# worm-privacy/proof-of-burn

Hardware: AMD Instinct MI355X
Metric: proof_of_burn witnesses/sec (higher is better)
Workload: dtype u64 bit-sliced lanes + BN254 Fr (8x32-bit Montgomery)

## Files before the change

### proof_of_burn_amd/csrc/poseidon_wide.hpp

```cpp
#pragma once
#include "kernels_common.hpp"

extern __shared__ uint32_t g_lds[];

#define POSW_NONE 0xFFFFFFFFu

template <bool RIDE, bool FAULT = false> struct PosWideT {
    __amdgpu_buffer_rsrc_t rs;
    uint32_t slot4;
    bool act;
    bool actb;
    const uint32_t* ktab;
    uint32_t kbase;
    uint32_t w_of_f;
    uint32_t w_also;
    mutable Fr pl, pv; mutable uint32_t pw, bad;
    uint32_t fault_f; bool fault_me;
    bool fault_val;
    __device__ __forceinline__ void ride_init() { pl = pv = fr_zero(); pw = 0; bad = 0xFFFFFFFFu; }
    __device__ __forceinline__ void ride_resolve() const { if (!fr_eq(pl, pv) && pw < bad) bad = pw; POB_OPAQUE(bad); }
    __device__ __forceinline__ Fr ld(uint32_t f) const {
        Fr v; const uint32_t off = act ? (f << 11) + slot4 : 0xFFFFF000u;
#pragma unroll
        for (int k = 0; k < 8; k++) v.l[k] = (uint32_t)__builtin_amdgcn_raw_buffer_load_b32(rs, (int)(off + 256u * k), 0, 0);
        return v;
    }
    __device__ __forceinline__ Fr st(bool on, uint32_t f, const Fr& v_in, bool also = false) const {
        const uint32_t off = on ? (f << 11) + slot4 : 0xFFFFF000u;
        Fr v = v_in;
        if constexpr (FAULT) { if (fault_val && fault_me && on && f == fault_f) v.l[0] ^= 1u; }
        const uint32_t flip = (FAULT && !fault_val && fault_me && f == fault_f) ? 1u : 0u;
#pragma unroll
        for (int k = 0; k < 8; k++) __builtin_amdgcn_raw_buffer_store_b32((int)(k == 0 ? v.l[0] ^ flip : v.l[k]), rs, (int)(off + 256u * k), 0, 0);
        if constexpr (RIDE) {
            Fr l;
#pragma unroll
            for (int k = 0; k < 8; k++) l.l[k] = (uint32_t)__builtin_amdgcn_raw_buffer_load_b32(rs, (int)(off + 256u * k), 0, 0);
            POB_RIDE_BARRIER();
            ride_resolve();
            pl = l; pv = fr_sel(on, v, fr_zero()); pw = also ? w_also : f + w_of_f;
        }
        return v;
    }
    __device__ __forceinline__ Fr kc(uint32_t idx) const {
        Fr v; const uint32_t* q = ktab + (size_t)(idx - kbase) * 8;
#pragma unroll
        for (int k = 0; k < 8; k++) v.l[k] = q[k];
        return v;
    }
};
typedef PosWideT<false> PosWide;
__device__ __forceinline__ Fr posw_from(const Fr& v, uint32_t src_lane) {
    Fr r;
#pragma unroll
    for (int k = 0; k < 8; k++) r.l[k] = (uint32_t)__builtin_amdgcn_ds_bpermute((int)(src_lane << 2), (int)v.l[k]);
    return r;
}
__device__ __forceinline__ Fr posw_group_sum(Fr v, uint32_t lane) {
#pragma unroll
    for (uint32_t m = 2; m >= 1; m >>= 1) v = fr_add(v, posw_from(v, lane ^ m));
    return v;
}

struct PosWDesc { uint32_t base, pre, in2, in3, in4, sub, also; };
template <int T, class PW> __device__ __forceinline__ Fr posw_input(const GArgs& A, const PosWDesc& d, const PW& W, uint32_t e, bool act) {
    Fr x = fr_zero();
    if (e == 1) x = A.L->prefix[d.pre];
    uint32_t a2 = e == 2 ? d.in2 : 0u, a3 = e == 3 ? d.in3 : 0u, a4 = e == 4 ? d.in4 : 0u;
    POB_OPAQUE(a2); POB_OPAQUE(a3); POB_OPAQUE(a4);
    const uint32_t aj = a2 | a3 | a4;
    const uint32_t src = (act && e >= 2) ? aj : POSW_NONE;
    PosWideT<false> Wi; Wi.rs = W.rs; Wi.slot4 = W.slot4; Wi.act = src != POSW_NONE;
    const Fr v = Wi.ld(src);
    if (src != POSW_NONE) x = v;
    const uint32_t sub = (act && e == (uint32_t)T - 1) ? d.sub : POSW_NONE;
    Wi.act = sub != POSW_NONE;
    const Fr s = Wi.ld(sub);
    if (sub != POSW_NONE) x = fr_sub(x, s);
    return fr_sel(act, x, fr_zero());
}

template <int T, class PW> __device__ __forceinline__ Fr posw_sbox(const PW& W, bool act, uint32_t e, Fr x, uint32_t off, uint32_t cr) {
    const Fr x2 = fr_sqr_inl(x), x4 = fr_sqr_inl(x2), x5 = fr_mul_inl(x4, x);
    const uint32_t sg = off + 4 * e;
    W.st(act, sg + 1, x); W.st(act, sg + 2, x2); W.st(act, sg + 3, x4); W.st(act, sg, x5);
    Fr y = fr_add(x5, W.kc(cr + (act ? e : 0)));
    W.st(act, off + 5 * T + e, x5); y = W.st(act, off + 4 * T + e, y);
    W.st(act, off + 7 * T + e, y);
    return y;
}
template <int T, class PW> __device__ __forceinline__ void posw_full(const PW& W, uint32_t lane, uint32_t j, Fr& x, Fr& xb, uint32_t off, uint32_t cr, uint32_t mat) {
    const bool act = W.act, actb = W.actb;
    const Fr y = posw_sbox<T>(W, act, j, x, off, cr);
    Fr yb = fr_zero();
    if constexpr (T == 5) yb = posw_sbox<T>(W, actb, 4, xb, off, cr);
    const uint32_t jc = act ? j : 0, g0 = lane & ~3u;
    Fr acc = fr_zero(), accb = fr_zero();
#pragma unroll 1
    for (uint32_t i = 0; i < (uint32_t)(T < 4 ? T : 4); i++) {
        const Fr yi = posw_from(y, g0 | i);
        acc = fr_add(acc, fr_mul_inl(W.kc(mat + jc * T + i), yi));
        if constexpr (T == 5) accb = fr_add(accb, fr_mul_inl(W.kc(mat + 4 * T + i), yi));
    }
    if constexpr (T == 5) {
        const Fr yi = posw_from(yb, g0 | 1u);
        acc = fr_add(acc, fr_mul_inl(W.kc(mat + jc * T + 4), yi));
        accb = fr_add(accb, fr_mul_inl(W.kc(mat + 4 * T + 4), yi));
        xb = W.st(actb, off + 6 * T + 4, accb);
    }
    x = W.st(act, off + 6 * T + j, acc);
}

template <int T, class PW> __device__ __forceinline__ void posw_run(const GArgs& A, const PosWDesc& d, const PW& W, uint32_t lane) {
    const PosOff k = pos_off(T);
    const uint32_t j = lane & 3u, base = d.base, g0 = lane & ~3u;
    const bool act = W.act, actb = W.actb, l0 = j == 0;
    const uint32_t jc = act ? j : 0;
    Fr x = posw_input<T>(A, d, W, j, act), xb = fr_zero();
    W.st(act && !l0, base + j, x);
    W.st(act && !l0, base + T + j, x);
    W.st(act && l0, base + 2 * T, x);
    W.st(act, base + 3 * T + 1 + j, x);
    x = fr_add(x, W.kc(k.C + jc));
    x = W.st(act, base + 2 * T + 1 + j, x);
    if constexpr (T == 5) {
        xb = posw_input<T>(A, d, W, 4, actb);
        W.st(actb, base + 4, xb); W.st(actb, base + T + 4, xb); W.st(actb, base + 3 * T + 5, xb);
        xb = fr_add(xb, W.kc(k.C + 4));
        xb = W.st(actb, base + 2 * T + 5, xb);
    }
    uint32_t off = base + 4 * T + 1;
#pragma unroll 1
    for (uint32_t r = 0; r < 4; r++) { posw_full<T>(W, lane, j, x, xb, off, k.C + (r + 1) * T, r == 3 ? k.Pm : k.M); off += 8 * T; }
    Fr pin0 = fr_zero();
    uint32_t poff = 0;
#pragma unroll 1
    for (uint32_t r = 0; r < (uint32_t)k.rp; r++) {
        const uint32_t sb = k.S + (2 * T - 1) * r;
        const Fr c1 = W.kc(sb + jc);
        const Fr m1 = fr_mul_inl(x, fr_sel(l0, x, c1));
        Fr m2, m3;
        if constexpr (T == 5) {
            const Fr cp = W.kc(r ? sb - (2 * T - 1) + T + 3 : sb);
            m2 = fr_mul_inl(fr_sel(l0, m1, pin0), fr_sel(l0, m1, cp));
            if (r) { xb = fr_add(xb, m2); xb = W.st(actb, poff + 4 + 4, xb); }
            m3 = fr_mul_inl(fr_sel(l0, m2, xb), fr_sel(l0, x, W.kc(sb + 4)));
        } else {
            m2 = fr_sqr_inl(m1);
            m3 = fr_mul_inl(m2, x);
        }
        const Fr s0 = fr_add(m3, W.kc(k.C + 5 * T + r));
        W.st(act && l0, off + 1, x); W.st(act && l0, off + 2, m1); W.st(act && l0, off + 3, m2); W.st(act && l0, off, m3);
        W.st(act, off + 4 + T + j, fr_sel(l0, s0, x));
        if constexpr (T == 5) W.st(actb, off + 4 + T + 4, xb);
        const Fr in0 = posw_from(s0, g0);
        const Fr c2 = W.kc(jc == 0 ? sb : sb + T + jc - 1);
        const Fr m4 = fr_mul_inl(c2, in0);
        Fr part = fr_sel(l0, m4, m1);
        if constexpr (T == 5) if (actb) part = fr_add(part, m3);
        if (!act) part = fr_zero();
        const Fr sum = posw_group_sum(part, lane);
        x = fr_sel(l0, sum, fr_add(x, m4));
        x = W.st(act, off + 4 + j, x);
        if constexpr (T == 5) { pin0 = in0; poff = off; }
        off += 4 + 2 * T;
    }
    if constexpr (T == 5) {
        xb = fr_add(xb, fr_mul_inl(pin0, W.kc(k.S + (2 * T - 1) * (k.rp - 1) + T + 3)));
        xb = W.st(actb, poff + 4 + 4, xb);
    }
#pragma unroll 1
    for (uint32_t r = 0; r < 3; r++) { posw_full<T>(W, lane, j, x, xb, off, k.C + 5 * T + k.rp + r * T, k.M); off += 8 * T; }
    {
        const Fr x2 = fr_sqr_inl(x), x4 = fr_sqr_inl(x2), x5 = fr_mul_inl(x4, x);
        const uint32_t sg = off + 4 * j;
        W.st(act, sg + 1, x); W.st(act, sg + 2, x2); W.st(act, sg + 3, x4); W.st(act, sg, x5);
        W.st(act, off + 4 * T + 1 + j, x5);
        Fr part = fr_mul_inl(W.kc(k.M + jc), x5);
        if constexpr (T == 5) {
            const Fr b2 = fr_sqr_inl(xb), b4 = fr_sqr_inl(b2), b5 = fr_mul_inl(b4, xb);
            W.st(actb, off + 17, xb); W.st(actb, off + 18, b2); W.st(actb, off + 19, b4); W.st(actb, off + 16, b5);
            W.st(actb, off + 4 * T + 5, b5);
            const Fr pb = fr_mul_inl(W.kc(k.M + 4), b5);
            if (actb) part = fr_add(part, pb);
        }
        if (!act) part = fr_zero();
        const Fr h = posw_group_sum(part, lane);
        W.st(act && l0, off + 4 * T, h);
        W.st(act && l0, base + T, h);
        W.st(act && l0, base, h);
        W.st(act && l0 && d.also != POSW_NONE, d.also, h, true);
    }
}

#define POSW_SLICES 4
#ifndef POSW_WAVES
#define POSW_WAVES 4
#endif
static_assert(POSW_SLICES % POSW_WAVES == 0, "the slices of a workgroup belong to one unit");
template <bool RIDE, bool FAULT = false> __device__ __forceinline__ void poswide_body(const GArgs& A, uint32_t bx, uint32_t g) {
    __builtin_amdgcn_s_setprio(3);
    const uint32_t lane = threadIdx.x & 63u;
    const UnitDesc* dp = A.units + POB_UNI(A.order[A.first + bx / POSW_SLICES]);
    const int T = (int)POB_UNI(dp->a[0]);
    const PosWDesc d = {POB_UNI(dp->cur.f), POB_UNI(dp->a[1]), POB_UNI(dp->a[2]), POB_UNI(dp->a[3]), POB_UNI(dp->a[4]), POB_UNI(dp->a[5]), POB_UNI(dp->a[6])};
    const PosOff k = pos_off(T);
    const uint32_t kend = T == 3 ? POS_OFF_C_4 : T == 4 ? POS_OFF_C_5 : POS_TABLE_LEN;
    for (uint32_t i = threadIdx.x; i < (kend - k.C) * 8; i += blockDim.x) g_lds[i] = A.pos_tab[(size_t)k.C * 8 + i];
    __syncthreads();
    PosWideT<RIDE, FAULT> W;
    uint32_t* frp = A.fr + (uint64_t)g * A.fr_stride;
    const uint64_t nf = A.fr_stride * 4;
    W.rs = __builtin_amdgcn_make_buffer_rsrc(frp, 0, (int)(nf > 0xFFFFF000ull ? 0xFFFFF000ull : nf), 0x00020000);
    const uint32_t slot = 16 * (bx % POSW_SLICES) + (lane >> 2);
    W.slot4 = slot * 4;
    W.act = (lane & 3u) < (uint32_t)T;
    W.actb = T == 5 && (lane & 3u) == 1;
    W.ktab = g_lds; W.kbase = k.C;
    W.w_of_f = POB_UNI(dp->cur.w) - d.base; W.w_also = POB_UNI(dp->cur.w);
    if constexpr (RIDE) W.ride_init();
    if constexpr (FAULT) { W.fault_f = A.fault_idx; W.fault_me = (A.fault_cls & 0xFFu) == 2 && g == A.fault_group && ((A.fault_lanes >> slot) & 1); W.fault_val = (A.fault_cls & FAULT_VALUE) != 0; }
    if (T == 3) posw_run<3>(A, d, W, lane); else if (T == 4) posw_run<4>(A, d, W, lane); else posw_run<5>(A, d, W, lane);
    if constexpr (RIDE) {
        W.ride_resolve();
        uint32_t b = W.bad;
#pragma unroll
        for (uint32_t m = 2; m >= 1; m >>= 1) { const uint32_t o = (uint32_t)__builtin_amdgcn_ds_bpermute((int)((lane ^ m) << 2), (int)b); b = o < b ? o : b; }
        if ((lane & 3u) == 0 && b != 0xFFFFFFFFu) atomicMin(&A.bad_wire[g * 64 + slot], b);
    }
}
template <bool RIDE, bool FAULT> __global__ void __launch_bounds__(64 * POSW_WAVES) k_poseidon_wide(GArgs A) { poswide_body<RIDE, FAULT>(A, POSW_WAVES * blockIdx.x + (threadIdx.x >> 6), blockIdx.y); }
static_assert(POS_TABLE_LEN - POS_OFF_C_5 >= POS_OFF_C_5 - POS_OFF_C_4 && POS_TABLE_LEN - POS_OFF_C_5 >= POS_OFF_C_4 - POS_OFF_C_3, "the T = 5 constants are the largest set");
#define POSW_LDS_BYTES ((POS_TABLE_LEN - POS_OFF_C_5) * 32u)
```

Before: 1.230 million.

## Batch Poseidon wide stores and readbacks through a four-slot ring, spread lane-4 work via DPP

Replaces the per-store write-then-readback verification with a 4-entry ring of pending stores. Readbacks are issued in batches and their comparisons resolved later, so load latency overlaps with the following arithmetic. The lone T=5 fifth-element lane's stores are redistributed across the quad using DPP quad permutes, so all four lanes issue stores in parallel instead of one lane serialising them. This adds register pressure from the ring state and intricate slot bookkeeping, and fault and ride-check attribution now depends on the ring indices being correct.

```diff
diff --git a/proof_of_burn_amd/csrc/poseidon_wide.hpp b/proof_of_burn_amd/csrc/poseidon_wide.hpp
--- a/proof_of_burn_amd/csrc/poseidon_wide.hpp
+++ b/proof_of_burn_amd/csrc/poseidon_wide.hpp
@@ -5,6 +5,8 @@
 
 #define POSW_NONE 0xFFFFFFFFu
 
+#define POSW_OFF 0xFFFFF000u
+#define POSW_RING 4
 template <bool RIDE, bool FAULT = false> struct PosWideT {
     __amdgpu_buffer_rsrc_t rs;
     uint32_t slot4;
@@ -14,33 +16,64 @@
     uint32_t kbase;
     uint32_t w_of_f;
     uint32_t w_also;
-    mutable Fr pl, pv; mutable uint32_t pw, bad;
+    mutable Fr pl[POSW_RING], pv[POSW_RING]; mutable uint32_t po[POSW_RING], bad;
     uint32_t fault_f; bool fault_me;
     bool fault_val;
-    __device__ __forceinline__ void ride_init() { pl = pv = fr_zero(); pw = 0; bad = 0xFFFFFFFFu; }
-    __device__ __forceinline__ void ride_resolve() const { if (!fr_eq(pl, pv) && pw < bad) bad = pw; POB_OPAQUE(bad); }
+    __device__ __forceinline__ void ride_init() {
+#pragma unroll
+        for (int i = 0; i < POSW_RING; i++) { pl[i] = pv[i] = fr_zero(); po[i] = POSW_OFF; }
+        bad = 0xFFFFFFFFu;
+    }
     __device__ __forceinline__ Fr ld(uint32_t f) const {
-        Fr v; const uint32_t off = act ? (f << 11) + slot4 : 0xFFFFF000u;
+        Fr v; const uint32_t off = act ? (f << 11) + slot4 : POSW_OFF;
 #pragma unroll
         for (int k = 0; k < 8; k++) v.l[k] = (uint32_t)__builtin_amdgcn_raw_buffer_load_b32(rs, (int)(off + 256u * k), 0, 0);
         return v;
     }
-    __device__ __forceinline__ Fr st(bool on, uint32_t f, const Fr& v_in, bool also = false) const {
-        const uint32_t off = on ? (f << 11) + slot4 : 0xFFFFF000u;
+    __device__ __forceinline__ Fr vf(bool on, uint32_t f, const Fr& v_in) const {
         Fr v = v_in;
         if constexpr (FAULT) { if (fault_val && fault_me && on && f == fault_f) v.l[0] ^= 1u; }
+        return v;
+    }
+    template <int I> __device__ __forceinline__ Fr put(bool on, uint32_t f, const Fr& v_in, bool pre = false) const {
+        static_assert(I >= 0 && I < POSW_RING, "slot index");
+        const uint32_t off = on ? (f << 11) + slot4 : POSW_OFF;
+        Fr v = v_in;
+        if constexpr (FAULT) { if (!pre) v = vf(on, f, v_in); }
         const uint32_t flip = (FAULT && !fault_val && fault_me && f == fault_f) ? 1u : 0u;
 #pragma unroll
         for (int k = 0; k < 8; k++) __builtin_amdgcn_raw_buffer_store_b32((int)(k == 0 ? v.l[0] ^ flip : v.l[k]), rs, (int)(off + 256u * k), 0, 0);
+        if constexpr (RIDE) { pv[I] = v; po[I] = off; }
+        return v;
+    }
+    template <int N> __device__ __forceinline__ void back() const {
         if constexpr (RIDE) {
-            Fr l;
-#pragma unroll
-            for (int k = 0; k < 8; k++) l.l[k] = (uint32_t)__builtin_amdgcn_raw_buffer_load_b32(rs, (int)(off + 256u * k), 0, 0);
+#pragma unroll
+            for (int i = 0; i < N; i++) {
+                uint32_t off = po[i]; POB_OPAQUE(off);
+#pragma unroll
+                for (int k = 0; k < 8; k++) pl[i].l[k] = (uint32_t)__builtin_amdgcn_raw_buffer_load_b32(rs, (int)(off + 256u * k), 0, 0);
+            }
             POB_RIDE_BARRIER();
-            ride_resolve();
-            pl = l; pv = fr_sel(on, v, fr_zero()); pw = also ? w_also : f + w_of_f;
-        }
-        return v;
+        }
+    }
+    template <int N, int ALSO = -1> __device__ __forceinline__ void resolve(bool al = false) const {
+        if constexpr (RIDE) {
+            POB_RIDE_BARRIER();
+#pragma unroll
+            for (int i = 0; i < N; i++) {
+                uint32_t w = (po[i] >> 11) + w_of_f;
+                if (i == ALSO && al) w = w_also;
+                if (po[i] != POSW_OFF && !fr_eq(pl[i], pv[i]) && w < bad) bad = w;
+            }
+            POB_OPAQUE(bad);
+        }
+    }
+    template <int FROM> __device__ __forceinline__ void idle() const {
+        if constexpr (RIDE) {
+#pragma unroll
+            for (int i = FROM; i < POSW_RING; i++) po[i] = POSW_OFF;
+        }
     }
     __device__ __forceinline__ Fr kc(uint32_t idx) const {
         Fr v; const uint32_t* q = ktab + (size_t)(idx - kbase) * 8;
@@ -56,6 +89,18 @@
     for (int k = 0; k < 8; k++) r.l[k] = (uint32_t)__builtin_amdgcn_ds_bpermute((int)(src_lane << 2), (int)v.l[k]);
     return r;
 }
+template <int Q> __device__ __forceinline__ Fr posw_quad(const Fr& v, uint32_t g0) {
+#ifdef POB_HOSTSIM
+    return posw_from(v, g0 | (uint32_t)Q);
+#else
+    Fr r; (void)g0;
+#pragma unroll
+    for (int k = 0; k < 8; k++) r.l[k] = (uint32_t)__builtin_amdgcn_update_dpp(0, (int)v.l[k], Q * 0x55, 0xF, 0xF, true);
+    return r;
+#endif
+}
+__device__ __forceinline__ uint32_t posw_pick(uint32_t j, uint32_t a, uint32_t b, uint32_t c, uint32_t d) { return j < 2 ? (j == 0 ? a : b) : (j == 2 ? c : d); }
+__device__ __forceinline__ Fr posw_pick(uint32_t j, const Fr& a, const Fr& b, const Fr& c, const Fr& d) { return fr_sel(j < 2, fr_sel(j == 0, a, b), fr_sel(j == 2, c, d)); }
 __device__ __forceinline__ Fr posw_group_sum(Fr v, uint32_t lane) {
 #pragma unroll
     for (uint32_t m = 2; m >= 1; m >>= 1) v = fr_add(v, posw_from(v, lane ^ m));
@@ -80,21 +125,34 @@
     return fr_sel(act, x, fr_zero());
 }
 
-template <int T, class PW> __device__ __forceinline__ Fr posw_sbox(const PW& W, bool act, uint32_t e, Fr x, uint32_t off, uint32_t cr) {
-    const Fr x2 = fr_sqr_inl(x), x4 = fr_sqr_inl(x2), x5 = fr_mul_inl(x4, x);
-    const uint32_t sg = off + 4 * e;
-    W.st(act, sg + 1, x); W.st(act, sg + 2, x2); W.st(act, sg + 3, x4); W.st(act, sg, x5);
-    Fr y = fr_add(x5, W.kc(cr + (act ? e : 0)));
-    W.st(act, off + 5 * T + e, x5); y = W.st(act, off + 4 * T + e, y);
-    W.st(act, off + 7 * T + e, y);
-    return y;
-}
 template <int T, class PW> __device__ __forceinline__ void posw_full(const PW& W, uint32_t lane, uint32_t j, Fr& x, Fr& xb, uint32_t off, uint32_t cr, uint32_t mat) {
-    const bool act = W.act, actb = W.actb;
-    const Fr y = posw_sbox<T>(W, act, j, x, off, cr);
-    Fr yb = fr_zero();
-    if constexpr (T == 5) yb = posw_sbox<T>(W, actb, 4, xb, off, cr);
-    const uint32_t jc = act ? j : 0, g0 = lane & ~3u;
+    const bool act = W.act, actb = W.actb, l1 = j == 1;
+    const uint32_t jc = act ? j : 0, g0 = lane & ~3u, sg = off + 4 * j;
+    const Fr x2 = fr_sqr_inl(x), x4 = fr_sqr_inl(x2);
+    Fr b4 = fr_zero();
+    W.template resolve<POSW_RING>();
+    W.template put<0>(act, sg + 1, x); W.template put<1>(act, sg + 2, x2); W.template put<2>(act, sg + 3, x4);
+    if constexpr (T == 5) {
+        const Fr b2 = fr_sqr_inl(xb);
+        b4 = fr_sqr_inl(b2);
+        W.template put<3>(!l1, posw_pick(j, off + 17, 0u, off + 18, off + 19), fr_sel(j == 0, posw_quad<1>(xb, g0), fr_sel(j == 2, posw_quad<1>(b2, g0), posw_quad<1>(b4, g0))));
+        W.template back<4>();
+    } else W.template back<3>();
+    if constexpr (T == 5) W.template resolve<4>();
+    const Fr x5 = fr_mul_inl(x4, x);
+    Fr y = fr_add(x5, W.kc(cr + jc));
+    Fr yb = fr_zero(), h2 = fr_zero();
+    if constexpr (T == 5) {
+        const Fr b5 = fr_mul_inl(b4, xb);
+        yb = W.vf(actb, off + 4 * T + 4, fr_add(b5, W.kc(cr + (actb ? 4u : 0u))));
+        h2 = fr_sel(j == 3, posw_quad<1>(yb, g0), posw_quad<1>(b5, g0));
+    }
+    if constexpr (T != 5) W.template resolve<3>();
+    W.template put<0>(act, sg, x5); W.template put<1>(act, off + 5 * T + j, x5);
+    y = W.template put<2>(act, off + 4 * T + j, y);
+    W.template put<3>(act, off + 7 * T + j, y);
+    W.template back<4>();
+    W.template resolve<4>();
     Fr acc = fr_zero(), accb = fr_zero();
 #pragma unroll 1
     for (uint32_t i = 0; i < (uint32_t)(T < 4 ? T : 4); i++) {
@@ -106,32 +164,39 @@
         const Fr yi = posw_from(yb, g0 | 1u);
         acc = fr_add(acc, fr_mul_inl(W.kc(mat + jc * T + 4), yi));
         accb = fr_add(accb, fr_mul_inl(W.kc(mat + 4 * T + 4), yi));
-        xb = W.st(actb, off + 6 * T + 4, accb);
-    }
-    x = W.st(act, off + 6 * T + j, acc);
+    }
+    x = W.template put<0>(act, off + 6 * T + j, acc);
+    if constexpr (T == 5) {
+        xb = W.template put<1>(true, posw_pick(j, off + 16, off + 6 * T + 4, off + 5 * T + 4, off + 7 * T + 4), fr_sel(l1, accb, h2));
+        W.template put<2>(actb, off + 4 * T + 4, yb, true);
+        W.template back<3>(); W.template idle<3>();
+    } else { W.template back<1>(); W.template idle<1>(); }
 }
 
 template <int T, class PW> __device__ __forceinline__ void posw_run(const GArgs& A, const PosWDesc& d, const PW& W, uint32_t lane) {
     const PosOff k = pos_off(T);
     const uint32_t j = lane & 3u, base = d.base, g0 = lane & ~3u;
-    const bool act = W.act, actb = W.actb, l0 = j == 0;
+    const bool act = W.act, actb = W.actb, l0 = j == 0, l1 = j == 1;
     const uint32_t jc = act ? j : 0;
     Fr x = posw_input<T>(A, d, W, j, act), xb = fr_zero();
-    W.st(act && !l0, base + j, x);
-    W.st(act && !l0, base + T + j, x);
-    W.st(act && l0, base + 2 * T, x);
-    W.st(act, base + 3 * T + 1 + j, x);
+    W.template put<0>(act, l0 ? base + 2 * T : base + j, x);
+    W.template put<1>(act && !l0, base + T + j, x);
+    W.template put<2>(act, base + 3 * T + 1 + j, x);
     x = fr_add(x, W.kc(k.C + jc));
-    x = W.st(act, base + 2 * T + 1 + j, x);
-    if constexpr (T == 5) {
-        xb = posw_input<T>(A, d, W, 4, actb);
-        W.st(actb, base + 4, xb); W.st(actb, base + T + 4, xb); W.st(actb, base + 3 * T + 5, xb);
-        xb = fr_add(xb, W.kc(k.C + 4));
-        xb = W.st(actb, base + 2 * T + 5, xb);
+    x = W.template put<3>(act, base + 2 * T + 1 + j, x);
+    W.template back<4>();
+    if constexpr (T == 5) {
+        const Fr i4 = posw_input<T>(A, d, W, 4, actb);
+        xb = W.vf(actb, base + 2 * T + 5, fr_add(i4, W.kc(k.C + 4)));
+        const Fr q4 = posw_quad<1>(i4, g0);
+        W.template resolve<4>();
+        W.template put<0>(true, posw_pick(j, base + 4, base + 2 * T + 5, base + T + 4, base + 3 * T + 5), fr_sel(l1, xb, q4), l1);
+        W.template back<1>(); W.template idle<1>();
     }
     uint32_t off = base + 4 * T + 1;
 #pragma unroll 1
     for (uint32_t r = 0; r < 4; r++) { posw_full<T>(W, lane, j, x, xb, off, k.C + (r + 1) * T, r == 3 ? k.Pm : k.M); off += 8 * T; }
+    constexpr int NP = T == 5 ? 4 : 3;
     Fr pin0 = fr_zero();
     uint32_t poff = 0;
 #pragma unroll 1
@@ -139,20 +204,26 @@
         const uint32_t sb = k.S + (2 * T - 1) * r;
         const Fr c1 = W.kc(sb + jc);
         const Fr m1 = fr_mul_inl(x, fr_sel(l0, x, c1));
+        W.template resolve<NP>();
         Fr m2, m3;
         if constexpr (T == 5) {
             const Fr cp = W.kc(r ? sb - (2 * T - 1) + T + 3 : sb);
             m2 = fr_mul_inl(fr_sel(l0, m1, pin0), fr_sel(l0, m1, cp));
-            if (r) { xb = fr_add(xb, m2); xb = W.st(actb, poff + 4 + 4, xb); }
+            if (r) xb = W.vf(actb, poff + 4 + 4, fr_add(xb, m2));
             m3 = fr_mul_inl(fr_sel(l0, m2, xb), fr_sel(l0, x, W.kc(sb + 4)));
         } else {
             m2 = fr_sqr_inl(m1);
             m3 = fr_mul_inl(m2, x);
         }
         const Fr s0 = fr_add(m3, W.kc(k.C + 5 * T + r));
-        W.st(act && l0, off + 1, x); W.st(act && l0, off + 2, m1); W.st(act && l0, off + 3, m2); W.st(act && l0, off, m3);
-        W.st(act, off + 4 + T + j, fr_sel(l0, s0, x));
-        if constexpr (T == 5) W.st(actb, off + 4 + T + 4, xb);
+        const Fr q1 = posw_quad<0>(m1, g0), q2 = posw_quad<0>(m2, g0);
+        if constexpr (T == 5) {
+            W.template put<0>(!l1 || r != 0, posw_pick(j, off + 1, poff + 4 + 4, off + 2, off + 3), posw_pick(j, x, xb, q1, q2), l1);
+            W.template put<1>(j < 2, l0 ? off : off + 4 + T + 4, fr_sel(l0, m3, xb));
+        } else {
+            W.template put<0>(true, posw_pick(j, off + 1, off + 2, off + 3, off), posw_pick(j, x, q1, q2, posw_quad<0>(m3, g0)));
+        }
+        W.template put<NP - 2>(act, off + 4 + T + j, fr_sel(l0, s0, x));
         const Fr in0 = posw_from(s0, g0);
         const Fr c2 = W.kc(jc == 0 ? sb : sb + T + jc - 1);
         const Fr m4 = fr_mul_inl(c2, in0);
@@ -161,35 +232,47 @@
         if (!act) part = fr_zero();
         const Fr sum = posw_group_sum(part, lane);
         x = fr_sel(l0, sum, fr_add(x, m4));
-        x = W.st(act, off + 4 + j, x);
+        x = W.template put<NP - 1>(act, off + 4 + j, x);
+        W.template back<NP>();
         if constexpr (T == 5) { pin0 = in0; poff = off; }
         off += 4 + 2 * T;
     }
     if constexpr (T == 5) {
         xb = fr_add(xb, fr_mul_inl(pin0, W.kc(k.S + (2 * T - 1) * (k.rp - 1) + T + 3)));
-        xb = W.st(actb, poff + 4 + 4, xb);
-    }
+        W.template resolve<NP>();
+        xb = W.template put<0>(actb, poff + 4 + 4, xb);
+        W.template back<1>(); W.template idle<1>();
+    } else W.template idle<NP>();
 #pragma unroll 1
     for (uint32_t r = 0; r < 3; r++) { posw_full<T>(W, lane, j, x, xb, off, k.C + 5 * T + k.rp + r * T, k.M); off += 8 * T; }
     {
-        const Fr x2 = fr_sqr_inl(x), x4 = fr_sqr_inl(x2), x5 = fr_mul_inl(x4, x);
+        const Fr x2 = fr_sqr_inl(x), x4 = fr_sqr_inl(x2);
         const uint32_t sg = off + 4 * j;
-        W.st(act, sg + 1, x); W.st(act, sg + 2, x2); W.st(act, sg + 3, x4); W.st(act, sg, x5);
-        W.st(act, off + 4 * T + 1 + j, x5);
+        Fr b5 = fr_zero();
+        W.template resolve<POSW_RING>();
+        W.template put<0>(act, sg + 1, x); W.template put<1>(act, sg + 2, x2); W.template put<2>(act, sg + 3, x4);
+        if constexpr (T == 5) {
+            const Fr b2 = fr_sqr_inl(xb), b4 = fr_sqr_inl(b2);
+            b5 = fr_mul_inl(b4, xb);
+            W.template put<3>(true, posw_pick(j, off + 18, off + 17, off + 19, off + 16), posw_pick(j, posw_quad<1>(b2, g0), xb, posw_quad<1>(b4, g0), posw_quad<1>(b5, g0)));
+            W.template back<4>();
+        } else W.template back<3>();
+        const Fr x5 = fr_mul_inl(x4, x);
         Fr part = fr_mul_inl(W.kc(k.M + jc), x5);
         if constexpr (T == 5) {
-            const Fr b2 = fr_sqr_inl(xb), b4 = fr_sqr_inl(b2), b5 = fr_mul_inl(b4, xb);
-            W.st(actb, off + 17, xb); W.st(actb, off + 18, b2); W.st(actb, off + 19, b4); W.st(actb, off + 16, b5);
-            W.st(actb, off + 4 * T + 5, b5);
             const Fr pb = fr_mul_inl(W.kc(k.M + 4), b5);
             if (actb) part = fr_add(part, pb);
         }
         if (!act) part = fr_zero();
+        W.template resolve<T == 5 ? 4 : 3>();
+        W.template put<0>(act, sg, x5);
+        W.template put<1>(act, off + 4 * T + 1 + j, x5);
+        if constexpr (T == 5) { W.template put<2>(actb, off + 4 * T + 5, b5); W.template back<3>(); } else W.template back<2>();
         const Fr h = posw_group_sum(part, lane);
-        W.st(act && l0, off + 4 * T, h);
-        W.st(act && l0, base + T, h);
-        W.st(act && l0, base, h);
-        W.st(act && l0 && d.also != POSW_NONE, d.also, h, true);
+        W.template resolve<T == 5 ? 3 : 2>();
+        W.template put<0>(j < 3 || d.also != POSW_NONE, posw_pick(j, off + 4 * T, base + T, base, d.also), h);
+        W.template back<1>();
+        W.template resolve<1, 0>(j == 3);
     }
 }
 
@@ -199,6 +282,9 @@
 #endif
 static_assert(POSW_SLICES % POSW_WAVES == 0, "the slices of a workgroup belong to one unit");
 template <bool RIDE, bool FAULT = false> __device__ __forceinline__ void poswide_body(const GArgs& A, uint32_t bx, uint32_t g) {
+#ifdef POSW_KNOCKOUT
+    return;
+#endif
     __builtin_amdgcn_s_setprio(3);
     const uint32_t lane = threadIdx.x & 63u;
     const UnitDesc* dp = A.units + POB_UNI(A.order[A.first + bx / POSW_SLICES]);
@@ -222,7 +308,6 @@
     if constexpr (FAULT) { W.fault_f = A.fault_idx; W.fault_me = (A.fault_cls & 0xFFu) == 2 && g == A.fault_group && ((A.fault_lanes >> slot) & 1); W.fault_val = (A.fault_cls & FAULT_VALUE) != 0; }
     if (T == 3) posw_run<3>(A, d, W, lane); else if (T == 4) posw_run<4>(A, d, W, lane); else posw_run<5>(A, d, W, lane);
     if constexpr (RIDE) {
-        W.ride_resolve();
         uint32_t b = W.bad;
 #pragma unroll
         for (uint32_t m = 2; m >= 1; m >>= 1) { const uint32_t o = (uint32_t)__builtin_amdgcn_ds_bpermute((int)((lane ^ m) << 2), (int)b); b = o < b ? o : b; }
```

Measured after the change: 1.263 million (median of 6 runs). 2.8% higher.
